# taishan1994/pytorch-distributed-NLP

Measured on AMD Instinct MI355X. Metric: samples_per_sec, higher is better.
Workload: dtype bf16; 1 GPU; model=bert-base, global_batch=32, seq_len=128, parallelism=dp1, physical_gpus=1, oversubscribed=False

## Files before the change

### pdnlp_amd/ops/csrc/embedding.hip

```cpp

#include <torch/extension.h>
#include <ATen/hip/HIPContext.h>

#include "common.h"

namespace {

template <typename T>
__global__ void emb_ln_fwd_kernel(
    const long* __restrict__ ids, const long* __restrict__ type_ids,
    const long* __restrict__ pos_ids, const T* __restrict__ word,
    const T* __restrict__ pos, const T* __restrict__ type_,
    const T* __restrict__ w, const T* __restrict__ b, T* __restrict__ y,
    float* __restrict__ mean_out, float* __restrict__ rstd_out, int H,
    float eps) {
  const int row = blockIdx.x;
  const int lane = threadIdx.x & (WAVE - 1);
  const T* wr = word + (long)ids[row] * H;
  const T* pr = pos + (long)pos_ids[row] * H;
  const T* tr = type_ + (long)type_ids[row] * H;
  T* yr = y + (long)row * H;

  const float shift = to_f32<T>(wr[0]) + to_f32<T>(pr[0]) + to_f32<T>(tr[0]);
  float sum = 0.f, sumsq = 0.f;
  for (int c = lane; c < H; c += WAVE) {
    const float v =
        to_f32<T>(wr[c]) + to_f32<T>(pr[c]) + to_f32<T>(tr[c]) - shift;
    sum += v;
    sumsq += v * v;
  }
  float md, mean, rstd;
  shifted_stats(wave_sum(sum), wave_sum(sumsq), shift, H, eps, md, mean, rstd);
  if (lane == 0) {
    mean_out[row] = mean;
    rstd_out[row] = rstd;
  }
  for (int c = lane; c < H; c += WAVE) {
    const float v = to_f32<T>(wr[c]) + to_f32<T>(pr[c]) + to_f32<T>(tr[c]);
    yr[c] = from_f32<T>((v - shift - md) * rstd * to_f32<T>(w[c]) +
                        to_f32<T>(b[c]));
  }
}

template <typename T>
__global__ void emb_ln_bwd_scatter_kernel(
    const T* __restrict__ dy, const long* __restrict__ ids,
    const long* __restrict__ type_ids, const long* __restrict__ pos_ids,
    const T* __restrict__ word, const T* __restrict__ pos,
    const T* __restrict__ type_, const T* __restrict__ w,
    const float* __restrict__ mean, const float* __restrict__ rstd,
    float* __restrict__ dword32, T* __restrict__ dsum_ws, int H) {
  const int row = blockIdx.x;
  const int lane = threadIdx.x & (WAVE - 1);
  const T* dyr = dy + (long)row * H;
  const T* wr = word + (long)ids[row] * H;
  const T* pr = pos + (long)pos_ids[row] * H;
  const T* tr = type_ + (long)type_ids[row] * H;
  const float mu = mean[row], rs = rstd[row];

  float s1 = 0.f, s2 = 0.f;
  for (int c = lane; c < H; c += WAVE) {
    const float dyw = to_f32<T>(dyr[c]) * to_f32<T>(w[c]);
    const float x = to_f32<T>(wr[c]) + to_f32<T>(pr[c]) + to_f32<T>(tr[c]);
    const float xh = (x - mu) * rs;
    s1 += dyw;
    s2 += dyw * xh;
  }
  s1 = wave_sum(s1) / H;
  s2 = wave_sum(s2) / H;
  float* dwr = dword32 + (long)ids[row] * H;
  for (int c = lane; c < H; c += WAVE) {
    const float dyw = to_f32<T>(dyr[c]) * to_f32<T>(w[c]);
    const float x = to_f32<T>(wr[c]) + to_f32<T>(pr[c]) + to_f32<T>(tr[c]);
    const float xh = (x - mu) * rs;
    const float dsum = rs * (dyw - s1 - xh * s2);
    atomicAdd(dwr + c, dsum);
    dsum_ws[(long)row * H + c] = from_f32<T>(dsum);
  }
}

template <typename T>
__global__ void emb_ln_bwd_small_table_kernel(
    const T* __restrict__ dsum_ws, const long* __restrict__ idx,
    float* __restrict__ dtab32, int R, int H, int rows_per_chunk,
    int tab_rows) {
  const int col = blockIdx.x * blockDim.x + threadIdx.x;
  if (col >= H) return;
  const int r0 = blockIdx.y * rows_per_chunk;
  const int r1 = min(r0 + rows_per_chunk, R);
  long cur = idx[r0];
  float acc = 0.f;
  for (int r = r0; r < r1; ++r) {
    const long v = idx[r];
    if (v != cur) {
      atomicAdd(dtab32 + cur * H + col, acc);
      cur = v;
      acc = 0.f;
    }
    acc += to_f32<T>(dsum_ws[(long)r * H + col]);
  }
  atomicAdd(dtab32 + cur * H + col, acc);
}

template <typename T>
__global__ void emb_ln_bwd_dwdb_kernel(
    const T* __restrict__ dy, const long* __restrict__ ids,
    const long* __restrict__ type_ids, const long* __restrict__ pos_ids,
    const T* __restrict__ word, const T* __restrict__ pos,
    const T* __restrict__ type_, const float* __restrict__ mean,
    const float* __restrict__ rstd, float* __restrict__ dlnw32,
    float* __restrict__ dlnb32, int R, int H, int rows_per_chunk) {
  const int col = blockIdx.x * blockDim.x + threadIdx.x;
  if (col >= H) return;
  const int r0 = blockIdx.y * rows_per_chunk;
  const int r1 = min(r0 + rows_per_chunk, R);
  float dw = 0.f, db = 0.f;
  for (int r = r0; r < r1; ++r) {
    const float d = to_f32<T>(dy[(long)r * H + col]);
    const float x = to_f32<T>(word[(long)ids[r] * H + col]) +
                    to_f32<T>(pos[(long)pos_ids[r] * H + col]) +
                    to_f32<T>(type_[(long)type_ids[r] * H + col]);
    const float xh = (x - mean[r]) * rstd[r];
    dw += d * xh;
    db += d;
  }
  atomicAdd(dlnw32 + col, dw);
  atomicAdd(dlnb32 + col, db);
}

}

std::vector<torch::Tensor> embedding_ln_fwd(
    torch::Tensor ids, torch::Tensor type_ids, torch::Tensor pos_ids,
    torch::Tensor word, torch::Tensor pos, torch::Tensor type_,
    torch::Tensor w, torch::Tensor b, double eps) {
  TORCH_CHECK(ids.is_cuda() && ids.scalar_type() == torch::kLong);
  const int H = word.size(1);
  const long R = ids.numel();
  auto y = torch::empty({ids.size(0), ids.size(1), H}, word.options());
  auto mean = torch::empty({R}, word.options().dtype(torch::kFloat32));
  auto rstd = torch::empty({R}, word.options().dtype(torch::kFloat32));
  auto stream = at::hip::getCurrentHIPStream();
  DISPATCH_FLOAT_TYPES(word.scalar_type(), "embedding_ln_fwd", [&] {
    hipLaunchKernelGGL((emb_ln_fwd_kernel<scalar_t>), dim3(R), dim3(WAVE), 0,
                       stream,
                       ids.data_ptr<long>(), type_ids.data_ptr<long>(),
                       pos_ids.data_ptr<long>(),
                       (const scalar_t*)word.data_ptr(),
                       (const scalar_t*)pos.data_ptr(),
                       (const scalar_t*)type_.data_ptr(),
                       (const scalar_t*)w.data_ptr(),
                       (const scalar_t*)b.data_ptr(), (scalar_t*)y.data_ptr(),
                       mean.data_ptr<float>(), rstd.data_ptr<float>(), H,
                       (float)eps);
  });
  return {y, mean, rstd};
}

std::vector<torch::Tensor> embedding_ln_bwd(
    torch::Tensor dy, torch::Tensor ids, torch::Tensor type_ids,
    torch::Tensor pos_ids, torch::Tensor word, torch::Tensor pos,
    torch::Tensor type_, torch::Tensor w, torch::Tensor mean,
    torch::Tensor rstd) {
  const int H = word.size(1);
  const long R = ids.numel();
  auto opts32 = word.options().dtype(torch::kFloat32);
  auto dword32 = torch::zeros({word.size(0), H}, opts32);
  auto dpos32 = torch::zeros({pos.size(0), H}, opts32);
  auto dtype32 = torch::zeros({type_.size(0), H}, opts32);
  auto dlnw32 = torch::zeros({H}, opts32);
  auto dlnb32 = torch::zeros({H}, opts32);
  auto dsum_ws = torch::empty({R, (long)H}, word.options());
  auto stream = at::hip::getCurrentHIPStream();
  const int rows_per_chunk = 16;
  const int chunks = (int)((R + rows_per_chunk - 1) / rows_per_chunk);
  DISPATCH_FLOAT_TYPES(word.scalar_type(), "embedding_ln_bwd", [&] {
    hipLaunchKernelGGL((emb_ln_bwd_scatter_kernel<scalar_t>), dim3(R),
                       dim3(WAVE), 0, stream,
                       (const scalar_t*)dy.data_ptr(), ids.data_ptr<long>(),
                       type_ids.data_ptr<long>(), pos_ids.data_ptr<long>(),
                       (const scalar_t*)word.data_ptr(),
                       (const scalar_t*)pos.data_ptr(),
                       (const scalar_t*)type_.data_ptr(),
                       (const scalar_t*)w.data_ptr(), mean.data_ptr<float>(),
                       rstd.data_ptr<float>(), dword32.data_ptr<float>(),
                       (scalar_t*)dsum_ws.data_ptr(), H);
    dim3 gridc((H + 255) / 256, chunks);
    hipLaunchKernelGGL((emb_ln_bwd_small_table_kernel<scalar_t>), gridc,
                       dim3(256), 0, stream,
                       (const scalar_t*)dsum_ws.data_ptr(),
                       pos_ids.data_ptr<long>(), dpos32.data_ptr<float>(),
                       (int)R, H, rows_per_chunk, (int)pos.size(0));
    hipLaunchKernelGGL((emb_ln_bwd_small_table_kernel<scalar_t>), gridc,
                       dim3(256), 0, stream,
                       (const scalar_t*)dsum_ws.data_ptr(),
                       type_ids.data_ptr<long>(), dtype32.data_ptr<float>(),
                       (int)R, H, rows_per_chunk, (int)type_.size(0));
    hipLaunchKernelGGL((emb_ln_bwd_dwdb_kernel<scalar_t>), gridc, dim3(256),
                       0, stream,
                       (const scalar_t*)dy.data_ptr(), ids.data_ptr<long>(),
                       type_ids.data_ptr<long>(), pos_ids.data_ptr<long>(),
                       (const scalar_t*)word.data_ptr(),
                       (const scalar_t*)pos.data_ptr(),
                       (const scalar_t*)type_.data_ptr(),
                       mean.data_ptr<float>(), rstd.data_ptr<float>(),
                       dlnw32.data_ptr<float>(), dlnb32.data_ptr<float>(),
                       (int)R, H, rows_per_chunk);
  });
  auto dt = word.scalar_type();
  return {dword32.to(dt), dpos32.to(dt), dtype32.to(dt), dlnw32.to(dt),
          dlnb32.to(dt)};
}
```

### pdnlp_amd/ops/csrc/gemm_tn.hip

```cpp

#include <torch/extension.h>
#include <ATen/hip/HIPContext.h>

#include <cstdlib>

#include "gemm_common.h"

namespace {

constexpr int NTHREADS = 256;
constexpr int BT = 64;
constexpr int BC = 64;

template <typename T, typename V8>
__global__ __launch_bounds__(NTHREADS)
void gemm_tn_kernel(const T* __restrict__ A, const T* __restrict__ B,
                    T* __restrict__ C, long M, long N, long K,
                    int tiles_k, int nwg) {
  const int wg = xcd_remap(blockIdx.x, nwg);
  const long n0 = (wg / tiles_k) * BT, k0 = (wg % tiles_k) * BT;

  __shared__ __attribute__((aligned(16))) char lds_a[2][BC * BT * 2];
  __shared__ __attribute__((aligned(16))) char lds_b[2][BC * BT * 2];

  const int wid = threadIdx.x >> 6;
  const int lane = threadIdx.x & (WAVE - 1);
  const int wr = (wid >> 1) * 32, wc = (wid & 1) * 32;

  f32x4 acc[2][2] = {};

  stage_tr<T, 4>(A, N, 0, M, n0, lds_a[0]);
  stage_tr<T, 4>(B, K, 0, M, k0, lds_b[0]);
  asm volatile("s_waitcnt vmcnt(0)" ::: "memory");
  __syncthreads();

  const int nchunks = (int)(M / BC);
  int cur = 0;
  for (int t = 0; t < nchunks; ++t) {
    if (t + 1 < nchunks) {
      stage_tr<T, 4>(A, N, (long)(t + 1) * BC, M, n0, lds_a[cur ^ 1]);
      stage_tr<T, 4>(B, K, (long)(t + 1) * BC, M, k0, lds_b[cur ^ 1]);
    }
#pragma unroll
    for (int ms = 0; ms < 2; ++ms) {
      V8 a_frag[2], b_frag[2];
      frag_tr4<V8>(frag_tr_base(lds_a[cur], wr, ms * 32),
                   frag_tr_base(lds_a[cur], wr + 16, ms * 32),
                   frag_tr_base(lds_b[cur], wc, ms * 32),
                   frag_tr_base(lds_b[cur], wc + 16, ms * 32),
                   a_frag, b_frag);
#pragma unroll
      for (int i = 0; i < 2; ++i) {
#pragma unroll
        for (int j = 0; j < 2; ++j) {
          acc[i][j] = mfma16<V8>(a_frag[i], b_frag[j], acc[i][j]);
        }
      }
    }
    asm volatile("s_waitcnt vmcnt(0)" ::: "memory");
    __syncthreads();
    cur ^= 1;
  }

  const int crow_off = (lane >> 4) * 4;
  const int ccol = lane & 15;
#pragma unroll
  for (int i = 0; i < 2; ++i) {
#pragma unroll
    for (int j = 0; j < 2; ++j) {
      const long k = k0 + wc + j * 16 + ccol;
      if (k >= K) continue;
#pragma unroll
      for (int r = 0; r < 4; ++r) {
        const long n = n0 + wr + i * 16 + crow_off + r;
        if (n >= N) continue;
        C[n * K + k] = from_f32<T>(acc[i][j][r]);
      }
    }
  }
}

template <typename T, typename V8>
__global__ __launch_bounds__(512)
void gemm_tn_w8_kernel(const T* __restrict__ A, const T* __restrict__ B,
                       T* __restrict__ C, long M, long N, long K,
                       int tiles_k, int nwg) {
  const int wg = xcd_remap(blockIdx.x, nwg);
  const long n0 = (wg / tiles_k) * BT, k0 = (wg % tiles_k) * BT;

  __shared__ __attribute__((aligned(16))) char lds_a[2][BC * BT * 2];
  __shared__ __attribute__((aligned(16))) char lds_b[2][BC * BT * 2];

  const int wid = threadIdx.x >> 6;
  const int lane = threadIdx.x & (WAVE - 1);
  const int wr = (wid >> 2) * 32, wc = (wid & 3) * 16;

  f32x4 acc[2] = {};

  stage_tr<T, 8>(A, N, 0, M, n0, lds_a[0]);
  stage_tr<T, 8>(B, K, 0, M, k0, lds_b[0]);
  asm volatile("s_waitcnt vmcnt(0)" ::: "memory");
  __syncthreads();

  const int nchunks = (int)(M / BC);
  int cur = 0;
  for (int t = 0; t < nchunks; ++t) {
    if (t + 1 < nchunks) {
      stage_tr<T, 8>(A, N, (long)(t + 1) * BC, M, n0, lds_a[cur ^ 1]);
      stage_tr<T, 8>(B, K, (long)(t + 1) * BC, M, k0, lds_b[cur ^ 1]);
    }
#pragma unroll
    for (int ms = 0; ms < 2; ++ms) {
      V8 a_frag[2];
      frag_tr2<V8>(frag_tr_base(lds_a[cur], wr, ms * 32),
                   frag_tr_base(lds_a[cur], wr + 16, ms * 32), a_frag);
      V8 b_frag = frag_tr1<V8>(frag_tr_base(lds_b[cur], wc, ms * 32));
#pragma unroll
      for (int i = 0; i < 2; ++i) {
        acc[i] = mfma16<V8>(a_frag[i], b_frag, acc[i]);
      }
    }
    asm volatile("s_waitcnt vmcnt(0)" ::: "memory");
    __syncthreads();
    cur ^= 1;
  }

  const int crow_off = (lane >> 4) * 4;
  const int ccol = lane & 15;
#pragma unroll
  for (int i = 0; i < 2; ++i) {
    const long k = k0 + wc + ccol;
    if (k >= K) continue;
#pragma unroll
    for (int r = 0; r < 4; ++r) {
      const long n = n0 + wr + i * 16 + crow_off + r;
      if (n >= N) continue;
      C[n * K + k] = from_f32<T>(acc[i][r]);
    }
  }
}

template <typename T, typename V8, bool RAWBAR, bool COLSUM>
__global__ __launch_bounds__(512)
void gemm_tn_sk_kernel(const T* __restrict__ A, const T* __restrict__ B,
                       float* __restrict__ P, long M, long N, long K,
                       int tiles_k, int ntiles, int sm, int nwg) {
  constexpr int BTN = 128, BTK = 128;
  constexpr int GLDS = 4;
  const int wg = xcd_remap(blockIdx.x, nwg);
  const int split = wg / ntiles;
  const int tile = wg % ntiles;
  const long n0 = (tile / tiles_k) * BTN, k0 = (tile % tiles_k) * BTK;
  const long mspan = M / sm;
  const long mbase = split * mspan;

  __shared__ __attribute__((aligned(16))) char lds_a[2][2 * 8192];
  __shared__ __attribute__((aligned(16))) char lds_b[2][2 * 8192];

  const int wid = threadIdx.x >> 6;
  const int lane = threadIdx.x & (WAVE - 1);
  const int wr = (wid >> 2) * 64, wc = (wid & 3) * 32;

  f32x4 acc[4][2] = {};
  const bool do_cs = COLSUM && k0 == 0;
  const int cs_q = wid & 3;
  f32x4 cs_acc = {};
  V8 ones;
#pragma unroll
  for (int e = 0; e < 8; ++e) ones[e] = 1.0f;

  auto stage = [&](long m_chunk, int buf) {
#pragma unroll
    for (int g = 0; g < 2; ++g) {
      stage_tr<T, 8>(A, N, m_chunk, M, n0 + g * 64, lds_a[buf] + g * 8192);
      stage_tr<T, 8>(B, K, m_chunk, M, k0 + g * 64, lds_b[buf] + g * 8192);
    }
  };

  stage(mbase, 0);
  if constexpr (!RAWBAR) {
    asm volatile("s_waitcnt vmcnt(0)" ::: "memory");
    __syncthreads();
  }

  const int nchunks = (int)(mspan / BC);
  int cur = 0;
  const int a_grp = wr >> 6;
  for (int t = 0; t < nchunks; ++t) {
    if (t + 1 < nchunks) stage(mbase + (long)(t + 1) * BC, cur ^ 1);
    if constexpr (RAWBAR) {
      if (t + 1 < nchunks)
        asm volatile("s_waitcnt vmcnt(%0) lgkmcnt(0)" ::"i"(GLDS)
                     : "memory");
      else
        asm volatile("s_waitcnt vmcnt(0) lgkmcnt(0)" ::: "memory");
      __builtin_amdgcn_s_barrier();
    }
#pragma unroll
    for (int ms = 0; ms < 2; ++ms) {
      V8 a_frag[4], b_frag[2];
#pragma unroll
      for (int i = 0; i < 4; i += 2)
        frag_tr2<V8>(
            frag_tr_base(lds_a[cur] + a_grp * 8192, (wr & 63) + i * 16,
                         ms * 32),
            frag_tr_base(lds_a[cur] + a_grp * 8192, (wr & 63) + (i + 1) * 16,
                         ms * 32),
            &a_frag[i]);
      {
        const int c0 = wc, c1 = wc + 16;
        frag_tr2<V8>(
            frag_tr_base(lds_b[cur] + (c0 >> 6) * 8192, c0 & 63, ms * 32),
            frag_tr_base(lds_b[cur] + (c1 >> 6) * 8192, c1 & 63, ms * 32),
            b_frag);
      }
      if constexpr (COLSUM) {
        if (do_cs) {
          typedef unsigned int u32x4 __attribute__((ext_vector_type(4)));
          u32x4 sel;
#pragma unroll
          for (int d = 0; d < 4; ++d) {
            const unsigned int f0 = reinterpret_cast<u32x4&>(a_frag[0])[d];
            const unsigned int f1 = reinterpret_cast<u32x4&>(a_frag[1])[d];
            const unsigned int f2 = reinterpret_cast<u32x4&>(a_frag[2])[d];
            const unsigned int f3 = reinterpret_cast<u32x4&>(a_frag[3])[d];
            const unsigned int lo = (cs_q & 1) ? f1 : f0;
            const unsigned int hi = (cs_q & 1) ? f3 : f2;
            sel[d] = (cs_q & 2) ? hi : lo;
          }
          const V8 av = reinterpret_cast<V8&>(sel);
          cs_acc = mfma16<V8>(av, ones, cs_acc);
        }
      }
#pragma unroll
      for (int i = 0; i < 4; ++i) {
#pragma unroll
        for (int j = 0; j < 2; ++j) {
          acc[i][j] = mfma16<V8>(a_frag[i], b_frag[j], acc[i][j]);
        }
      }
    }
    if constexpr (RAWBAR) {
      asm volatile("s_waitcnt lgkmcnt(0)" ::: "memory");
      __builtin_amdgcn_s_barrier();
    } else {
      asm volatile("s_waitcnt vmcnt(0)" ::: "memory");
      __syncthreads();
    }
    cur ^= 1;
  }

  float* Pout = P + (long)split * N * K;
  const int crow_off = (lane >> 4) * 4;
  const int ccol = lane & 15;
#pragma unroll
  for (int i = 0; i < 4; ++i) {
#pragma unroll
    for (int j = 0; j < 2; ++j) {
      const long k = k0 + wc + j * 16 + ccol;
      if (k >= K) continue;
#pragma unroll
      for (int r = 0; r < 4; ++r) {
        const long n = n0 + wr + i * 16 + crow_off + r;
        if (n >= N) continue;
        Pout[n * K + k] = acc[i][j][r];
      }
    }
  }
  if constexpr (COLSUM) {
    if (do_cs && ccol == 0) {
      float* PS = P + (long)sm * N * K + (long)split * N;
#pragma unroll
      for (int r = 0; r < 4; ++r) {
        const long n = n0 + wr + cs_q * 16 + crow_off + r;
        if (n < N) PS[n] = cs_acc[r];
      }
    }
  }
}

template <typename T>
__device__ __forceinline__ void fold_partials4(const float* __restrict__ P,
                                               T* __restrict__ C, long i4,
                                               long NK, int sm) {
  typedef float f4 __attribute__((ext_vector_type(4)));
  f4 acc = *reinterpret_cast<const f4*>(P + i4);
  for (int s = 1; s < sm; ++s) {
    f4 v = *reinterpret_cast<const f4*>(P + (long)s * NK + i4);
#pragma unroll
    for (int q = 0; q < 4; ++q) acc[q] += v[q];
  }
#pragma unroll
  for (int q = 0; q < 4; ++q) C[i4 + q] = from_f32<T>(acc[q]);
}

template <typename T>
__global__ __launch_bounds__(256)
void reduce_partials_kernel(const float* __restrict__ P, T* __restrict__ C,
                            long NK, int sm) {
  const long i4 = ((long)blockIdx.x * 256 + threadIdx.x) * 4;
  if (i4 >= NK) return;
  fold_partials4<T>(P, C, i4, NK, sm);
}

template <typename T>
__global__ __launch_bounds__(256)
void reduce_partials_colsum_kernel(const float* __restrict__ P,
                                   T* __restrict__ C, T* __restrict__ CS,
                                   long NK, long N, int sm, int rblocks) {
  if ((int)blockIdx.x < rblocks) {
    const long i4 = ((long)blockIdx.x * 256 + threadIdx.x) * 4;
    if (i4 >= NK) return;
    fold_partials4<T>(P, C, i4, NK, sm);
  } else {
    const long i4 = ((long)(blockIdx.x - rblocks) * 256 + threadIdx.x) * 4;
    if (i4 >= N) return;
    fold_partials4<T>(P + (long)sm * NK, CS, i4, N, sm);
  }
}

int tn_v2_split(long M, int tiles2) {
  int sm = 1;
  if (const char* env = getenv("PDNLP_TN_SM")) sm = atoi(env);
  else if (tiles2 < 512)
    sm = tiles2 <= 108 ? 4 : 2;
  if (sm < 1) sm = 1;
  while (sm > 1 && M % (64L * sm) != 0) sm /= 2;
  return sm;
}

bool tn_v2_ok(long N, long K) {
  return getenv("PDNLP_TN_V1") == nullptr && N % 128 == 0 && K % 128 == 0;
}

template <typename T, typename V8>
void launch_tn_v2(const torch::Tensor& A, const torch::Tensor& B,
                  torch::Tensor& P, torch::Tensor& C, torch::Tensor& CS,
                  long M, long N, long K, int tiles2, int sm, bool colsum,
                  bool sync, hipStream_t stream) {
  const int nwg2 = tiles2 * sm;
  const long NK = N * K;
  const int rblocks = (int)((NK / 4 + 255) / 256);
  auto kernel =
      colsum ? (sync ? gemm_tn_sk_kernel<T, V8, false, true>
                     : gemm_tn_sk_kernel<T, V8, true, true>)
             : (sync ? gemm_tn_sk_kernel<T, V8, false, false>
                     : gemm_tn_sk_kernel<T, V8, true, false>);
  hipLaunchKernelGGL(kernel, dim3(nwg2), dim3(512), 0, stream,
                     (const T*)A.data_ptr(), (const T*)B.data_ptr(),
                     (float*)P.data_ptr(), M, N, K, (int)(K / 128), tiles2,
                     sm, nwg2);
  if (colsum) {
    const int cblocks = (int)((N / 4 + 255) / 256);
    hipLaunchKernelGGL((reduce_partials_colsum_kernel<T>),
                       dim3(rblocks + cblocks), dim3(256), 0, stream,
                       (const float*)P.data_ptr(), (T*)C.data_ptr(),
                       (T*)CS.data_ptr(), NK, N, sm, rblocks);
  } else {
    hipLaunchKernelGGL((reduce_partials_kernel<T>), dim3(rblocks), dim3(256),
                       0, stream, (const float*)P.data_ptr(),
                       (T*)C.data_ptr(), NK, sm);
  }
}

template <typename T, typename V8>
void launch_tn_64(const torch::Tensor& A, const torch::Tensor& B,
                  torch::Tensor& C, long M, long N, long K,
                  hipStream_t stream) {
  const int tiles_k = (int)((K + BT - 1) / BT);
  const int nwg = (int)((N + BT - 1) / BT) * tiles_k;
  const bool w8 = getenv("PDNLP_TN_W4") == nullptr;
  auto kernel = w8 ? gemm_tn_w8_kernel<T, V8> : gemm_tn_kernel<T, V8>;
  hipLaunchKernelGGL(kernel, dim3(nwg), dim3(w8 ? 512 : NTHREADS), 0, stream,
                     (const T*)A.data_ptr(), (const T*)B.data_ptr(),
                     (T*)C.data_ptr(), M, N, K, tiles_k, nwg);
}

}

torch::Tensor col_sum(torch::Tensor x);

namespace {

std::pair<torch::Tensor, torch::Tensor> tn_impl(const torch::Tensor& A,
                                                const torch::Tensor& B,
                                                bool colsum) {
  TORCH_CHECK(A.is_cuda() && A.is_contiguous() && B.is_contiguous());
  TORCH_CHECK(A.dim() == 2 && B.dim() == 2 && A.size(0) == B.size(0));
  const long M = A.size(0), N = A.size(1), K = B.size(1);
  TORCH_CHECK(M % BC == 0, "gemm_tn: M must be a multiple of 64");
  TORCH_CHECK(N % 64 == 0 && K % 64 == 0,
              "gemm_tn: N and K must be multiples of 64");
  const bool bf16 = A.scalar_type() == torch::kBFloat16;
  TORCH_CHECK(bf16 || A.scalar_type() == torch::kHalf,
              "gemm_tn: bf16/fp16 only");
  TORCH_CHECK(A.scalar_type() == B.scalar_type(),
              "gemm_tn: A and B dtypes differ");
  auto C = torch::empty({N, K}, A.options());
  torch::Tensor CS;
  auto stream = at::hip::getCurrentHIPStream();
  if (!tn_v2_ok(N, K)) {
    if (bf16) launch_tn_64<__hip_bfloat16, bf16x8>(A, B, C, M, N, K, stream);
    else launch_tn_64<__half, f16x8>(A, B, C, M, N, K, stream);
    if (colsum) CS = col_sum(A);
    return {C, CS};
  }
  const int tiles2 = (int)((N / 128) * (K / 128));
  const int sm = tn_v2_split(M, tiles2);
  auto P = torch::empty({(long)sm * (N * K + (colsum ? N : 0))},
                        A.options().dtype(torch::kFloat32));
  if (colsum) CS = torch::empty({N}, A.options());
  const bool sync = getenv("PDNLP_TN_SYNC") != nullptr || (!colsum && !bf16);
  if (bf16)
    launch_tn_v2<__hip_bfloat16, bf16x8>(A, B, P, C, CS, M, N, K, tiles2, sm,
                                         colsum, sync, stream);
  else
    launch_tn_v2<__half, f16x8>(A, B, P, C, CS, M, N, K, tiles2, sm, colsum,
                                sync, stream);
  return {C, CS};
}

}

torch::Tensor gemm_tn(torch::Tensor A, torch::Tensor B) {
  return tn_impl(A, B, false).first;
}

std::vector<torch::Tensor> gemm_tn_colsum(torch::Tensor A, torch::Tensor B) {
  auto r = tn_impl(A, B, true);
  return {r.first, r.second};
}
```

Measured before the change: 4540 samples/s.

## Replace embedding backward atomics with indexed gather-sum and fuse split-K fold into GEMM

The embedding+LayerNorm backward now writes per-row gradients to an fp32 workspace, builds a per-table-row count and head index, and sums contributing rows with a gather, splitting heavily used rows into chunks that are folded afterwards. This replaces float atomic scatter into full fp32 tables and the dtype-conversion copies. The dLN weight/bias kernel is vectorised with an LDS reduction and per-chunk partials instead of atomics. Separately, the split-K TN GEMM gains an in-kernel fold: the last workgroup per tile, chosen through a per-stream persistent counter, sums the partial slabs and writes bf16 output directly, which removes the separate reduce kernel but adds counter state and more complex synchronisation.

```diff
diff --git a/pdnlp_amd/ops/csrc/embedding.hip b/pdnlp_amd/ops/csrc/embedding.hip
--- a/pdnlp_amd/ops/csrc/embedding.hip
+++ b/pdnlp_amd/ops/csrc/embedding.hip
@@ -1,6 +1,8 @@
 
 #include <torch/extension.h>
 #include <ATen/hip/HIPContext.h>
+
+#include <climits>
 
 #include "common.h"
 
@@ -42,16 +44,40 @@
   }
 }
 
-template <typename T>
-__global__ void emb_ln_bwd_scatter_kernel(
+
+constexpr int EMB_LIST_MAX = 1024;
+
+struct EmbTabs {
+  const long* idx0; const long* idx1; const long* idx2;
+  void* out0; void* out1; void* out2;
+  int rows0, rows1, rows2;
+};
+
+struct EmbIndex {
+  int* count;
+  int* head;
+  int* nheavy;
+  int* heavy;
+  int D, ch, nch, maxslot;
+};
+
+template <typename T>
+__global__ void emb_ln_bwd_row_kernel(
     const T* __restrict__ dy, const long* __restrict__ ids,
     const long* __restrict__ type_ids, const long* __restrict__ pos_ids,
     const T* __restrict__ word, const T* __restrict__ pos,
     const T* __restrict__ type_, const T* __restrict__ w,
     const float* __restrict__ mean, const float* __restrict__ rstd,
-    float* __restrict__ dword32, T* __restrict__ dsum_ws, int H) {
+    float* __restrict__ ws, EmbIndex ix, int H) {
   const int row = blockIdx.x;
   const int lane = threadIdx.x & (WAVE - 1);
+  for (long i = (long)row * WAVE + lane; i < ix.D;
+       i += (long)gridDim.x * WAVE) {
+    ix.count[i] = 0;
+    ix.head[i] = INT_MAX;
+  }
+  if (row == 0 && lane == 0) *ix.nheavy = 0;
+
   const T* dyr = dy + (long)row * H;
   const T* wr = word + (long)ids[row] * H;
   const T* pr = pos + (long)pos_ids[row] * H;
@@ -68,64 +94,243 @@
   }
   s1 = wave_sum(s1) / H;
   s2 = wave_sum(s2) / H;
-  float* dwr = dword32 + (long)ids[row] * H;
   for (int c = lane; c < H; c += WAVE) {
     const float dyw = to_f32<T>(dyr[c]) * to_f32<T>(w[c]);
     const float x = to_f32<T>(wr[c]) + to_f32<T>(pr[c]) + to_f32<T>(tr[c]);
     const float xh = (x - mu) * rs;
-    const float dsum = rs * (dyw - s1 - xh * s2);
-    atomicAdd(dwr + c, dsum);
-    dsum_ws[(long)row * H + c] = from_f32<T>(dsum);
-  }
-}
-
-template <typename T>
-__global__ void emb_ln_bwd_small_table_kernel(
-    const T* __restrict__ dsum_ws, const long* __restrict__ idx,
-    float* __restrict__ dtab32, int R, int H, int rows_per_chunk,
-    int tab_rows) {
-  const int col = blockIdx.x * blockDim.x + threadIdx.x;
+    ws[(long)row * H + c] = rs * (dyw - s1 - xh * s2);
+  }
+}
+
+__global__ __launch_bounds__(256)
+void emb_ln_bwd_index_kernel(EmbTabs tb, EmbIndex ix, int R) {
+  const int lane = threadIdx.x & (WAVE - 1);
+  const int r = blockIdx.x * blockDim.x + threadIdx.x;
+  const int t = blockIdx.y;
+  const long* idx = t == 0 ? tb.idx0 : t == 1 ? tb.idx1 : tb.idx2;
+  const int rows = t == 0 ? tb.rows0 : t == 1 ? tb.rows1 : tb.rows2;
+  const int off = t == 0 ? 0 : t == 1 ? tb.rows0 : tb.rows0 + tb.rows1;
+  long v = -1;
+  if (r < R) v = idx[r];
+  const bool valid = v >= 0 && v < rows;
+  const int d = off + (int)v;
+  bool leader = false;
+  int n = 0;
+  unsigned long long todo = __ballot(valid);
+  while (todo) {
+    const int l = __ffsll((long long)todo) - 1;
+    const int dl = __shfl(d, l, WAVE);
+    const unsigned long long m = __ballot(valid && d == dl);
+    if (lane == l) {
+      leader = true;
+      n = __popcll(m);
+    }
+    todo &= ~m;
+  }
+  if (leader) {
+    const int old = atomicAdd(ix.count + d, n);
+    atomicMin(ix.head + d, r);
+    if (old <= ix.ch && old + n > ix.ch) {
+      const int s = atomicAdd(ix.nheavy, 1);
+      if (s < ix.maxslot) ix.heavy[s] = d;
+    }
+  }
+}
+
+__device__ __forceinline__ void emb_dest(const EmbTabs& tb, int d,
+                                         const long*& idx, long& v,
+                                         void*& out) {
+  if (d < tb.rows0) {
+    idx = tb.idx0; v = d; out = tb.out0;
+  } else if (d < tb.rows0 + tb.rows1) {
+    idx = tb.idx1; v = d - tb.rows0; out = tb.out1;
+  } else {
+    idx = tb.idx2; v = d - tb.rows0 - tb.rows1; out = tb.out2;
+  }
+}
+
+typedef float emb_f4 __attribute__((ext_vector_type(4)));
+
+template <typename T>
+__device__ __forceinline__ emb_f4 emb_sum_rows(const float* __restrict__ ws,
+                                               const int* list, int n, int H,
+                                               int col, bool round_t) {
+  emb_f4 acc = {0.f, 0.f, 0.f, 0.f};
+  for (int k = 0; k < n; k += 8) {
+    emb_f4 v[8];
+#pragma unroll
+    for (int j = 0; j < 8; ++j) {
+      const int row = list[min(k + j, n - 1)];
+      v[j] = *reinterpret_cast<const emb_f4*>(ws + (long)row * H + col);
+    }
+#pragma unroll
+    for (int j = 0; j < 8; ++j) {
+      const bool keep = k + j < n;
+#pragma unroll
+      for (int q = 0; q < 4; ++q) {
+        float x = v[j][q];
+        if (round_t) x = to_f32<T>(from_f32<T>(x));
+        acc[q] += keep ? x : 0.f;
+      }
+    }
+  }
+  return acc;
+}
+
+template <typename T>
+__device__ __forceinline__ void emb_store_row(void* out, long v, int H,
+                                              int col, emb_f4 acc) {
+  v4_t<T> o;
+#pragma unroll
+  for (int q = 0; q < 4; ++q) set_elem<T>(o, q, acc[q]);
+  st4<T>((T*)out + v * H + col, o);
+}
+
+template <typename T>
+__global__ void emb_ln_bwd_sum_kernel(const float* __restrict__ ws,
+                                      EmbTabs tb, EmbIndex ix,
+                                      float* __restrict__ part, int R,
+                                      int H) {
+  __shared__ int list[EMB_LIST_MAX];
+  __shared__ int nlist;
+  const int lane = threadIdx.x & (WAVE - 1);
+  const int col = (threadIdx.x >> 6) * 256 + lane * 4;
+  const bool colok = col < H;
+  const int nitems = ix.maxslot * ix.nch;
+  const bool item = (int)blockIdx.x < nitems;
+
+  int d, r0, r1, want;
+  long pslab = 0;
+  if (item) {
+    const int s = blockIdx.x / ix.nch, c = blockIdx.x % ix.nch;
+    if (s >= min(*ix.nheavy, ix.maxslot)) return;
+    d = ix.heavy[s];
+    r0 = c * ix.ch;
+    r1 = min(R, r0 + ix.ch);
+    want = ix.ch;
+    pslab = (long)blockIdx.x * H;
+  } else {
+    d = blockIdx.x - nitems;
+    want = ix.count[d];
+    if (want > ix.ch) return;
+    r0 = ix.head[d];
+    r1 = R;
+  }
+  const long* idx;
+  long v;
+  void* out;
+  emb_dest(tb, d, idx, v, out);
+  if (want == 0) {
+    if (colok) emb_store_row<T>(out, v, H, col, emb_f4{0.f, 0.f, 0.f, 0.f});
+    return;
+  }
+
+  if (threadIdx.x < WAVE) {
+    int found = 0;
+    if (!item && want == 1) {
+      if (lane == 0) list[0] = r0;
+      found = 1;
+    } else {
+      for (int base = r0; base < r1 && found < want; base += 4 * WAVE) {
+        long x[4];
+#pragma unroll
+        for (int j = 0; j < 4; ++j) {
+          const int r = base + j * WAVE + lane;
+          x[j] = idx[min(r, r1 - 1)];
+        }
+#pragma unroll
+        for (int j = 0; j < 4; ++j) {
+          const int r = base + j * WAVE + lane;
+          const bool hit = r < r1 && x[j] == v;
+          const unsigned long long m = __ballot(hit);
+          const int at = found + __popcll(m & ((1ull << lane) - 1ull));
+          if (hit && at < EMB_LIST_MAX) list[at] = r;
+          found += __popcll(m);
+        }
+      }
+    }
+    if (lane == 0) nlist = min(found, EMB_LIST_MAX);
+  }
+  __syncthreads();
+  if (!colok) return;
+  const emb_f4 acc = emb_sum_rows<T>(ws, list, nlist, H, col, d >= tb.rows0);
+  if (item)
+    *reinterpret_cast<emb_f4*>(part + pslab + col) = acc;
+  else
+    emb_store_row<T>(out, v, H, col, acc);
+}
+
+template <typename T>
+__global__ void emb_ln_bwd_fold_kernel(const float* __restrict__ part,
+                                       EmbTabs tb, EmbIndex ix, int H) {
+  const int s = blockIdx.x;
+  if (s >= min(*ix.nheavy, ix.maxslot)) return;
+  const int col = (threadIdx.x >> 6) * 256 + (threadIdx.x & (WAVE - 1)) * 4;
   if (col >= H) return;
-  const int r0 = blockIdx.y * rows_per_chunk;
-  const int r1 = min(r0 + rows_per_chunk, R);
-  long cur = idx[r0];
-  float acc = 0.f;
-  for (int r = r0; r < r1; ++r) {
-    const long v = idx[r];
-    if (v != cur) {
-      atomicAdd(dtab32 + cur * H + col, acc);
-      cur = v;
-      acc = 0.f;
-    }
-    acc += to_f32<T>(dsum_ws[(long)r * H + col]);
-  }
-  atomicAdd(dtab32 + cur * H + col, acc);
-}
-
-template <typename T>
-__global__ void emb_ln_bwd_dwdb_kernel(
+  const long* idx;
+  long v;
+  void* out;
+  emb_dest(tb, ix.heavy[s], idx, v, out);
+  const float* p = part + (long)s * ix.nch * H + col;
+  emb_f4 acc = {0.f, 0.f, 0.f, 0.f};
+#pragma unroll 8
+  for (int c = 0; c < ix.nch; ++c) {
+    const emb_f4 x = *reinterpret_cast<const emb_f4*>(p + (long)c * H);
+#pragma unroll
+    for (int q = 0; q < 4; ++q) acc[q] += x[q];
+  }
+  emb_store_row<T>(out, v, H, col, acc);
+}
+
+template <typename T>
+__global__ __launch_bounds__(256)
+void emb_ln_bwd_dwdb_kernel(
     const T* __restrict__ dy, const long* __restrict__ ids,
     const long* __restrict__ type_ids, const long* __restrict__ pos_ids,
     const T* __restrict__ word, const T* __restrict__ pos,
     const T* __restrict__ type_, const float* __restrict__ mean,
-    const float* __restrict__ rstd, float* __restrict__ dlnw32,
-    float* __restrict__ dlnb32, int R, int H, int rows_per_chunk) {
-  const int col = blockIdx.x * blockDim.x + threadIdx.x;
-  if (col >= H) return;
+    const float* __restrict__ rstd, float* __restrict__ part, int R, int H,
+    int rows_per_chunk) {
+  __shared__ float lds[16][2][64];
+  const int quad = threadIdx.x & 15;
+  const int strip = threadIdx.x >> 4;
+  const int c0 = blockIdx.x * 64 + quad * 4;
   const int r0 = blockIdx.y * rows_per_chunk;
   const int r1 = min(r0 + rows_per_chunk, R);
-  float dw = 0.f, db = 0.f;
-  for (int r = r0; r < r1; ++r) {
-    const float d = to_f32<T>(dy[(long)r * H + col]);
-    const float x = to_f32<T>(word[(long)ids[r] * H + col]) +
-                    to_f32<T>(pos[(long)pos_ids[r] * H + col]) +
-                    to_f32<T>(type_[(long)type_ids[r] * H + col]);
-    const float xh = (x - mean[r]) * rstd[r];
-    dw += d * xh;
-    db += d;
-  }
-  atomicAdd(dlnw32 + col, dw);
-  atomicAdd(dlnb32 + col, db);
+  float dw[4] = {}, db[4] = {};
+  if (c0 < H) {
+    for (int r = r0 + strip; r < r1; r += 16) {
+      const float mu = mean[r], rs = rstd[r];
+      const v4_t<T> dv = ld4(dy + (long)r * H + c0);
+      const v4_t<T> wv = ld4(word + (long)ids[r] * H + c0);
+      const v4_t<T> pv = ld4(pos + (long)pos_ids[r] * H + c0);
+      const v4_t<T> tv = ld4(type_ + (long)type_ids[r] * H + c0);
+#pragma unroll
+      for (int j = 0; j < 4; ++j) {
+        const float d = elem<T>(dv, j);
+        const float x = elem<T>(wv, j) + elem<T>(pv, j) + elem<T>(tv, j);
+        const float xh = (x - mu) * rs;
+        dw[j] += d * xh;
+        db[j] += d;
+      }
+    }
+  }
+#pragma unroll
+  for (int j = 0; j < 4; ++j) {
+    lds[strip][0][quad * 4 + j] = dw[j];
+    lds[strip][1][quad * 4 + j] = db[j];
+  }
+  __syncthreads();
+  if (threadIdx.x < 2 * 64) {
+    const int kind = threadIdx.x >> 6, colb = threadIdx.x & 63;
+    const int gc = blockIdx.x * 64 + colb;
+    if (gc < H) {
+      float s = 0.f;
+#pragma unroll
+      for (int st = 0; st < 16; ++st) s += lds[st][kind][colb];
+      part[(long)blockIdx.y * 2 * H + kind * H + gc] = s;
+    }
+  }
 }
 
 }
@@ -164,50 +369,82 @@
     torch::Tensor rstd) {
   const int H = word.size(1);
   const long R = ids.numel();
+  TORCH_CHECK(H % 4 == 0 && H <= 4096,
+              "embedding_ln_bwd: hidden size must be a multiple of 4, <= 4096");
+  TORCH_CHECK(R > 0 && R < INT_MAX / WAVE, "embedding_ln_bwd: bad row count");
+  TORCH_CHECK(ids.is_contiguous() && type_ids.is_contiguous() &&
+              pos_ids.is_contiguous() && dy.is_contiguous());
+  const long D = word.size(0) + pos.size(0) + type_.size(0);
+  TORCH_CHECK(D < INT_MAX, "embedding_ln_bwd: tables too large");
+
+  EmbIndex ix;
+  ix.ch = (int)std::min<long>(EMB_LIST_MAX, std::max<long>(128, (R + 31) / 32));
+  ix.nch = (int)((R + ix.ch - 1) / ix.ch);
+  ix.maxslot = 3 * ix.nch;
+  ix.D = (int)D;
+
   auto opts32 = word.options().dtype(torch::kFloat32);
-  auto dword32 = torch::zeros({word.size(0), H}, opts32);
-  auto dpos32 = torch::zeros({pos.size(0), H}, opts32);
-  auto dtype32 = torch::zeros({type_.size(0), H}, opts32);
-  auto dlnw32 = torch::zeros({H}, opts32);
-  auto dlnb32 = torch::zeros({H}, opts32);
-  auto dsum_ws = torch::empty({R, (long)H}, word.options());
+  auto ws = torch::empty({R, (long)H}, opts32);
+  auto ibuf = torch::empty({2 * D + 1 + ix.maxslot},
+                           word.options().dtype(torch::kInt32));
+  auto part = torch::empty({(long)ix.maxslot * ix.nch, (long)H}, opts32);
+  const int rows_per_chunk = (int)((R + 31) / 32);
+  const int chunks = (int)((R + rows_per_chunk - 1) / rows_per_chunk);
+  auto cpart = torch::empty({(long)chunks, 2L, (long)H}, opts32);
+  auto dword = torch::empty({word.size(0), (long)H}, word.options());
+  auto dpos = torch::empty({pos.size(0), (long)H}, word.options());
+  auto dtype_ = torch::empty({type_.size(0), (long)H}, word.options());
+  auto dln = torch::empty({2L, (long)H}, word.options());
+
+  ix.count = ibuf.data_ptr<int>();
+  ix.head = ix.count + D;
+  ix.nheavy = ix.head + D;
+  ix.heavy = ix.nheavy + 1;
+  EmbTabs tb;
+  tb.idx0 = ids.data_ptr<long>();
+  tb.idx1 = pos_ids.data_ptr<long>();
+  tb.idx2 = type_ids.data_ptr<long>();
+  tb.out0 = dword.data_ptr();
+  tb.out1 = dpos.data_ptr();
+  tb.out2 = dtype_.data_ptr();
+  tb.rows0 = (int)word.size(0);
+  tb.rows1 = (int)pos.size(0);
+  tb.rows2 = (int)type_.size(0);
+
   auto stream = at::hip::getCurrentHIPStream();
-  const int rows_per_chunk = 16;
-  const int chunks = (int)((R + rows_per_chunk - 1) / rows_per_chunk);
+  const int ncg = (H + 255) / 256;
   DISPATCH_FLOAT_TYPES(word.scalar_type(), "embedding_ln_bwd", [&] {
-    hipLaunchKernelGGL((emb_ln_bwd_scatter_kernel<scalar_t>), dim3(R),
-                       dim3(WAVE), 0, stream,
+    hipLaunchKernelGGL((emb_ln_bwd_row_kernel<scalar_t>), dim3(R), dim3(WAVE),
+                       0, stream,
                        (const scalar_t*)dy.data_ptr(), ids.data_ptr<long>(),
                        type_ids.data_ptr<long>(), pos_ids.data_ptr<long>(),
                        (const scalar_t*)word.data_ptr(),
                        (const scalar_t*)pos.data_ptr(),
                        (const scalar_t*)type_.data_ptr(),
                        (const scalar_t*)w.data_ptr(), mean.data_ptr<float>(),
-                       rstd.data_ptr<float>(), dword32.data_ptr<float>(),
-                       (scalar_t*)dsum_ws.data_ptr(), H);
-    dim3 gridc((H + 255) / 256, chunks);
-    hipLaunchKernelGGL((emb_ln_bwd_small_table_kernel<scalar_t>), gridc,
-                       dim3(256), 0, stream,
-                       (const scalar_t*)dsum_ws.data_ptr(),
-                       pos_ids.data_ptr<long>(), dpos32.data_ptr<float>(),
-                       (int)R, H, rows_per_chunk, (int)pos.size(0));
-    hipLaunchKernelGGL((emb_ln_bwd_small_table_kernel<scalar_t>), gridc,
-                       dim3(256), 0, stream,
-                       (const scalar_t*)dsum_ws.data_ptr(),
-                       type_ids.data_ptr<long>(), dtype32.data_ptr<float>(),
-                       (int)R, H, rows_per_chunk, (int)type_.size(0));
-    hipLaunchKernelGGL((emb_ln_bwd_dwdb_kernel<scalar_t>), gridc, dim3(256),
-                       0, stream,
+                       rstd.data_ptr<float>(), ws.data_ptr<float>(), ix, H);
+    hipLaunchKernelGGL(emb_ln_bwd_index_kernel, dim3((R + 255) / 256, 3),
+                       dim3(256), 0, stream, tb, ix, (int)R);
+    hipLaunchKernelGGL((emb_ln_bwd_sum_kernel<scalar_t>),
+                       dim3(ix.maxslot * ix.nch + (int)D), dim3(WAVE * ncg), 0,
+                       stream, ws.data_ptr<float>(), tb, ix,
+                       part.data_ptr<float>(), (int)R, H);
+    hipLaunchKernelGGL((emb_ln_bwd_fold_kernel<scalar_t>), dim3(ix.maxslot),
+                       dim3(WAVE * ncg), 0, stream, part.data_ptr<float>(),
+                       tb, ix, H);
+    hipLaunchKernelGGL((emb_ln_bwd_dwdb_kernel<scalar_t>),
+                       dim3((H + 63) / 64, chunks), dim3(256), 0, stream,
                        (const scalar_t*)dy.data_ptr(), ids.data_ptr<long>(),
                        type_ids.data_ptr<long>(), pos_ids.data_ptr<long>(),
                        (const scalar_t*)word.data_ptr(),
                        (const scalar_t*)pos.data_ptr(),
                        (const scalar_t*)type_.data_ptr(),
                        mean.data_ptr<float>(), rstd.data_ptr<float>(),
-                       dlnw32.data_ptr<float>(), dlnb32.data_ptr<float>(),
-                       (int)R, H, rows_per_chunk);
+                       cpart.data_ptr<float>(), (int)R, H, rows_per_chunk);
+    hipLaunchKernelGGL((reduce_cols_cast_kernel<scalar_t>),
+                       dim3((2 * H + 63) / 64), dim3(256), 0, stream,
+                       cpart.data_ptr<float>(), (scalar_t*)dln.data_ptr(),
+                       (long)(2 * H), chunks);
   });
-  auto dt = word.scalar_type();
-  return {dword32.to(dt), dpos32.to(dt), dtype32.to(dt), dlnw32.to(dt),
-          dlnb32.to(dt)};
-}
+  return {dword, dpos, dtype_, dln[0], dln[1]};
+}
diff --git a/pdnlp_amd/ops/csrc/gemm_tn.hip b/pdnlp_amd/ops/csrc/gemm_tn.hip
--- a/pdnlp_amd/ops/csrc/gemm_tn.hip
+++ b/pdnlp_amd/ops/csrc/gemm_tn.hip
@@ -3,6 +3,8 @@
 #include <ATen/hip/HIPContext.h>
 
 #include <cstdlib>
+#include <mutex>
+#include <unordered_map>
 
 #include "gemm_common.h"
 
@@ -140,11 +142,13 @@
   }
 }
 
-template <typename T, typename V8, bool RAWBAR, bool COLSUM>
+template <typename T, typename V8, bool RAWBAR, bool COLSUM, bool FOLD>
 __global__ __launch_bounds__(512)
 void gemm_tn_sk_kernel(const T* __restrict__ A, const T* __restrict__ B,
-                       float* __restrict__ P, long M, long N, long K,
-                       int tiles_k, int ntiles, int sm, int nwg) {
+                       float* __restrict__ P, T* __restrict__ C,
+                       T* __restrict__ CS, unsigned int* __restrict__ cnt,
+                       long M, long N, long K, int tiles_k, int ntiles,
+                       int sm, int nwg) {
   constexpr int BTN = 128, BTK = 128;
   constexpr int GLDS = 4;
   const int wg = xcd_remap(blockIdx.x, nwg);
@@ -250,30 +254,121 @@
     cur ^= 1;
   }
 
-  float* Pout = P + (long)split * N * K;
   const int crow_off = (lane >> 4) * 4;
   const int ccol = lane & 15;
-#pragma unroll
-  for (int i = 0; i < 4; ++i) {
-#pragma unroll
-    for (int j = 0; j < 2; ++j) {
-      const long k = k0 + wc + j * 16 + ccol;
-      if (k >= K) continue;
-#pragma unroll
-      for (int r = 0; r < 4; ++r) {
-        const long n = n0 + wr + i * 16 + crow_off + r;
-        if (n >= N) continue;
-        Pout[n * K + k] = acc[i][j][r];
-      }
-    }
-  }
   if constexpr (COLSUM) {
     if (do_cs && ccol == 0) {
       float* PS = P + (long)sm * N * K + (long)split * N;
 #pragma unroll
       for (int r = 0; r < 4; ++r) {
         const long n = n0 + wr + cs_q * 16 + crow_off + r;
-        if (n < N) PS[n] = cs_acc[r];
+        if (n >= N) continue;
+        if constexpr (FOLD)
+          __hip_atomic_store(PS + n, cs_acc[r], __ATOMIC_RELAXED,
+                             __HIP_MEMORY_SCOPE_AGENT);
+        else
+          PS[n] = cs_acc[r];
+      }
+    }
+  }
+  if constexpr (!FOLD) {
+    float* Pout = P + (long)split * N * K;
+#pragma unroll
+    for (int i = 0; i < 4; ++i) {
+#pragma unroll
+      for (int j = 0; j < 2; ++j) {
+        const long k = k0 + wc + j * 16 + ccol;
+        if (k >= K) continue;
+#pragma unroll
+        for (int r = 0; r < 4; ++r) {
+          const long n = n0 + wr + i * 16 + crow_off + r;
+          if (n >= N) continue;
+          Pout[n * K + k] = acc[i][j][r];
+        }
+      }
+    }
+  } else {
+    constexpr long SLAB = (long)BTN * BTK;
+    typedef unsigned int u32x4 __attribute__((ext_vector_type(4)));
+    const int foff = (wid * 8 * WAVE + lane) * 16;
+    auto slab_rsrc = [&](int s) {
+      return __builtin_amdgcn_make_buffer_rsrc(
+          P + ((long)s * ntiles + tile) * SLAB, 0, (int)(SLAB * 4),
+          0x00020000);
+    };
+    {
+      const auto rs = slab_rsrc(split);
+#pragma unroll
+      for (int i = 0; i < 4; ++i) {
+#pragma unroll
+        for (int j = 0; j < 2; ++j)
+          __builtin_amdgcn_raw_buffer_store_b128(
+              reinterpret_cast<const u32x4&>(acc[i][j]), rs,
+              foff + (i * 2 + j) * WAVE * 16, 0,  16);
+      }
+    }
+    asm volatile("s_waitcnt vmcnt(0)" ::: "memory");
+    __syncthreads();
+    unsigned int* lds_ticket = reinterpret_cast<unsigned int*>(&lds_b[0][0]);
+    if (threadIdx.x == 0)
+      *lds_ticket = __builtin_amdgcn_atomic_inc32(
+          cnt + tile, (unsigned int)(sm - 1), __ATOMIC_RELAXED, "agent");
+    __syncthreads();
+    if (*lds_ticket != (unsigned int)(sm - 1)) return;
+
+    auto get_slab = [&](int s, f32x4 (&v)[8]) {
+      if (s == split) {
+#pragma unroll
+        for (int f = 0; f < 8; ++f) v[f] = acc[f >> 1][f & 1];
+      } else {
+        const auto rs = slab_rsrc(s);
+#pragma unroll
+        for (int f = 0; f < 8; ++f) {
+          const u32x4 x = __builtin_amdgcn_raw_buffer_load_b128(
+              rs, foff + f * WAVE * 16, 0,  16);
+          v[f] = reinterpret_cast<const f32x4&>(x);
+        }
+      }
+    };
+    f32x4 sum[8];
+    get_slab(0, sum);
+    for (int s = 1; s < sm; ++s) {
+      f32x4 v[8];
+      get_slab(s, v);
+#pragma unroll
+      for (int f = 0; f < 8; ++f) {
+#pragma unroll
+        for (int q = 0; q < 4; ++q) sum[f][q] += v[f][q];
+      }
+    }
+    T* lds_c = reinterpret_cast<T*>(&lds_a[0][0]);
+#pragma unroll
+    for (int i = 0; i < 4; ++i) {
+#pragma unroll
+      for (int j = 0; j < 2; ++j) {
+#pragma unroll
+        for (int r = 0; r < 4; ++r)
+          lds_c[(wr + i * 16 + crow_off + r) * BTK + wc + j * 16 + ccol] =
+              from_f32<T>(sum[i * 2 + j][r]);
+      }
+    }
+    __syncthreads();
+#pragma unroll
+    for (int it = 0; it < 4; ++it) {
+      const int q = it * 512 + threadIdx.x;
+      const int row = q >> 4, c8 = (q & 15) * 8;
+      *reinterpret_cast<u32x4*>(C + (n0 + row) * K + k0 + c8) =
+          *reinterpret_cast<const u32x4*>(lds_c + row * BTK + c8);
+    }
+    if constexpr (COLSUM) {
+      if (do_cs && threadIdx.x < BTN) {
+        const float* PS = P + (long)sm * N * K + n0 + threadIdx.x;
+        float a = __hip_atomic_load(PS, __ATOMIC_RELAXED,
+                                    __HIP_MEMORY_SCOPE_AGENT);
+        for (int s = 1; s < sm; ++s)
+          a += __hip_atomic_load(PS + (long)s * N, __ATOMIC_RELAXED,
+                                 __HIP_MEMORY_SCOPE_AGENT);
+        CS[n0 + threadIdx.x] = from_f32<T>(a);
       }
     }
   }
@@ -333,23 +428,63 @@
   return getenv("PDNLP_TN_V1") == nullptr && N % 128 == 0 && K % 128 == 0;
 }
 
+constexpr int TN_CNT_TILES = 4096;
+constexpr int TN_CNT_SLOTS = 16;
+
+struct TnCounters {
+  torch::Tensor buf;
+  std::unordered_map<hipStream_t, int> slot;
+};
+
+unsigned int* tn_fold_counters(const torch::Tensor& like, hipStream_t stream,
+                               int tiles2) {
+  if (tiles2 > TN_CNT_TILES) return nullptr;
+  static std::mutex mu;
+  static auto* pool = new std::unordered_map<int, TnCounters>();
+  std::lock_guard<std::mutex> lock(mu);
+  hipStreamCaptureStatus cap = hipStreamCaptureStatusNone;
+  HIP_CHECK(hipStreamIsCapturing(stream, &cap));
+  const int dev = like.get_device();
+  auto it = pool->find(dev);
+  if (it == pool->end()) {
+    if (cap != hipStreamCaptureStatusNone) return nullptr;
+    TnCounters c;
+    c.buf = torch::zeros({(long)TN_CNT_SLOTS * TN_CNT_TILES},
+                         like.options().dtype(torch::kInt32));
+    HIP_CHECK(hipStreamSynchronize(stream));
+    it = pool->emplace(dev, std::move(c)).first;
+  }
+  auto& c = it->second;
+  auto st = c.slot.find(stream);
+  if (st == c.slot.end()) {
+    if ((int)c.slot.size() >= TN_CNT_SLOTS) return nullptr;
+    st = c.slot.emplace(stream, (int)c.slot.size()).first;
+  }
+  return reinterpret_cast<unsigned int*>(c.buf.data_ptr<int>()) +
+         (long)st->second * TN_CNT_TILES;
+}
+
 template <typename T, typename V8>
 void launch_tn_v2(const torch::Tensor& A, const torch::Tensor& B,
                   torch::Tensor& P, torch::Tensor& C, torch::Tensor& CS,
                   long M, long N, long K, int tiles2, int sm, bool colsum,
-                  bool sync, hipStream_t stream) {
+                  bool sync, unsigned int* cnt, hipStream_t stream) {
   const int nwg2 = tiles2 * sm;
   const long NK = N * K;
   const int rblocks = (int)((NK / 4 + 255) / 256);
-  auto kernel =
-      colsum ? (sync ? gemm_tn_sk_kernel<T, V8, false, true>
-                     : gemm_tn_sk_kernel<T, V8, true, true>)
-             : (sync ? gemm_tn_sk_kernel<T, V8, false, false>
-                     : gemm_tn_sk_kernel<T, V8, true, false>);
-  hipLaunchKernelGGL(kernel, dim3(nwg2), dim3(512), 0, stream,
-                     (const T*)A.data_ptr(), (const T*)B.data_ptr(),
-                     (float*)P.data_ptr(), M, N, K, (int)(K / 128), tiles2,
-                     sm, nwg2);
+  DISPATCH_BOOL(cnt != nullptr, FOLD, [&] {
+    auto kernel =
+        colsum ? (sync ? gemm_tn_sk_kernel<T, V8, false, true, FOLD>
+                       : gemm_tn_sk_kernel<T, V8, true, true, FOLD>)
+               : (sync ? gemm_tn_sk_kernel<T, V8, false, false, FOLD>
+                       : gemm_tn_sk_kernel<T, V8, true, false, FOLD>);
+    hipLaunchKernelGGL(kernel, dim3(nwg2), dim3(512), 0, stream,
+                       (const T*)A.data_ptr(), (const T*)B.data_ptr(),
+                       (float*)P.data_ptr(), (T*)C.data_ptr(),
+                       colsum ? (T*)CS.data_ptr() : nullptr, cnt, M, N, K,
+                       (int)(K / 128), tiles2, sm, nwg2);
+  });
+  if (cnt != nullptr) return;
   if (colsum) {
     const int cblocks = (int)((N / 4 + 255) / 256);
     hipLaunchKernelGGL((reduce_partials_colsum_kernel<T>),
@@ -411,12 +546,15 @@
                         A.options().dtype(torch::kFloat32));
   if (colsum) CS = torch::empty({N}, A.options());
   const bool sync = getenv("PDNLP_TN_SYNC") != nullptr || (!colsum && !bf16);
+  unsigned int* cnt = getenv("PDNLP_TN_FOLD2") != nullptr
+                          ? nullptr
+                          : tn_fold_counters(A, stream, tiles2);
   if (bf16)
     launch_tn_v2<__hip_bfloat16, bf16x8>(A, B, P, C, CS, M, N, K, tiles2, sm,
-                                         colsum, sync, stream);
+                                         colsum, sync, cnt, stream);
   else
     launch_tn_v2<__half, f16x8>(A, B, P, C, CS, M, N, K, tiles2, sm, colsum,
-                                sync, stream);
+                                sync, cnt, stream);
   return {C, CS};
 }
 
```

New measurement: 4643 samples/s (median of 6 runs). 1.02x the previous value.
